# tianyili2017/HEVC-Complexity-Reduction

Measured on AMD Instinct MI355X. Metric: CTUs/sec (ETH-CNN inference), higher is better.
Workload: dtype f32; 1 GPU; All-Intra 3840x2160 QP32, 50 frames synthetic YUV; width=3840, height=2160, frames_per_gpu=50, qp=32, ranks=1, devices_visible=1, rank0_device=0, one_rank_per_device=True, device=AMD Radeon Graphics (gfx950:sramecc+:xnack-, 256 CUs), host NUMA node 0

## Files before the change

hevc-complexity-reduction_amd/csrc/ethcnn_context.cpp:

```cpp
#include "ethcnn_ctx.h"

static thread_local std::string g_create_err;

int set_err(ethcnn_ctx* c, int code, const char* fmt, ...) {
    char buf[512];
    va_list ap;
    va_start(ap, fmt);
    std::vsnprintf(buf, sizeof buf, fmt, ap);
    va_end(ap);
    if (c) c->err = buf; else g_create_err = buf;
    return code;
}

extern "C" const char* ethcnn_version(void) { return "ethcnn-mi355x 0.1 (gfx950)"; }

extern "C" const char* ethcnn_last_error(const ethcnn_ctx* ctx) {
    return ctx ? ctx->err.c_str() : g_create_err.c_str();
}

int ensure_side_streams(ethcnn_ctx* c) {
    hipStream_t* ss[] = {&c->copy_in, &c->copy_out, &c->s_tile};
    for (hipStream_t* s : ss)
        if (!*s) HIPCHK(c, hipStreamCreateWithFlags(s, hipStreamNonBlocking));
    return 0;
}

static void free_workspace(ethcnn_ctx* c) {
    Workspace& w = c->ws;
    void* ptrs[] = {w.featb, w.xs, w.xm, w.xl, w.feat, w.h1, w.h2, w.logits, w.raw, w.flags, c->xs1, c->xm1, c->xl1, c->h1_1, c->flags1};
    for (void* p : ptrs)
        if (p) (void)hipFree(p);
    w = Workspace();
    c->xs1 = c->xm1 = c->xl1 = nullptr;
    c->h1_1 = nullptr;
    c->flags1 = nullptr;
}

Workspace ws_view(const ethcnn_ctx* c, int p) {
    Workspace v = c->ws;
    if (p) {
        v.xs = c->xs1;
        v.xm = c->xm1;
        v.xl = c->xl1;
        v.h1 = c->h1_1;
        v.flags = c->flags1;
    }
    return v;
}

int ensure_workspace(ethcnn_ctx* c, int n, int chunks) {
    Workspace& w = c->ws;
    const int cap = (n + 15) / 16 * 16;
    if (cap > w.cap) {
        free_workspace(c);
        HIPCHK(c, hipMalloc((void**)&w.xs, (size_t)cap * 4096));
        HIPCHK(c, hipMalloc((void**)&w.xm, (size_t)cap * 2048));
        HIPCHK(c, hipMalloc((void**)&w.xl, (size_t)cap * 512));
        HIPCHK(c, hipMalloc((void**)&w.feat, (size_t)cap * kNFeat * 4));
        HIPCHK(c, hipMalloc((void**)&w.h1, (size_t)cap * kNVec * 4));
        HIPCHK(c, hipMalloc((void**)&w.h2, (size_t)cap * kNFc2 * 4));
        HIPCHK(c, hipMalloc((void**)&w.logits, (size_t)cap * kNOut * 4));
        HIPCHK(c, hipMalloc((void**)&w.raw, (size_t)cap * kNOut * 4));
        HIPCHK(c, hipMalloc((void**)&c->xs1, (size_t)cap * 4096));
        HIPCHK(c, hipMalloc((void**)&c->xm1, (size_t)cap * 2048));
        HIPCHK(c, hipMalloc((void**)&c->xl1, (size_t)cap * 512));
        HIPCHK(c, hipMalloc((void**)&c->h1_1, (size_t)cap * kNVec * 4));
        w.cap = cap;
    }
    if (c->fc1_plan != 0 && !w.featb)
        HIPCHK(c, hipMalloc((void**)&w.featb, (size_t)((w.cap + 31) / 32) * kFastPairBytes));
    const int words = sync_words(chunks);
    if (words > w.flags_cap) {
        if (w.flags) (void)hipFree(w.flags);
        if (c->flags1) (void)hipFree(c->flags1);
        w.flags = c->flags1 = nullptr;
        w.flags_cap = 0;
        HIPCHK(c, hipMalloc((void**)&w.flags, (size_t)words * sizeof(int)));
        HIPCHK(c, hipMalloc((void**)&c->flags1, (size_t)words * sizeof(int)));
        w.flags_cap = words;
    }
    return 0;
}

extern "C" int ethcnn_create(ethcnn_ctx** out, const ethcnn_options* opt) {
    if (!out) return set_err(nullptr, ETHCNN_ERR_ARG, "ethcnn_create: out is NULL");
    *out = nullptr;
    const auto t_enter = std::chrono::steady_clock::now();
    int ndev = 0;
    hipError_t e = hipGetDeviceCount(&ndev);
    const auto t_runtime = std::chrono::steady_clock::now();
    if (e != hipSuccess || ndev <= 0)
        return set_err(nullptr, ETHCNN_ERR_DEVICE, "no HIP device available (%s): libethcnn has no CPU fallback",
                       e == hipSuccess ? "device count 0" : hipGetErrorString(e));
    const int dev = opt ? opt->device : 0;
    if (dev < 0 || dev >= ndev) return set_err(nullptr, ETHCNN_ERR_ARG, "device %d out of range (0..%d)", dev, ndev - 1);
    std::vector<std::pair<const char*, std::chrono::steady_clock::time_point>> marks;
    auto mark = [&](const char* what) { marks.emplace_back(what, std::chrono::steady_clock::now()); };
    hipDeviceProp_t prop;
    if ((e = hipGetDeviceProperties(&prop, dev)) != hipSuccess)
        return set_err(nullptr, ETHCNN_ERR_DEVICE, "hipGetDeviceProperties: %s", hipGetErrorString(e));
    if (std::strncmp(prop.gcnArchName, "gfx950", 6) != 0)
        return set_err(nullptr, ETHCNN_ERR_DEVICE, "device %d is %s; libethcnn is built for gfx950 only", dev, prop.gcnArchName);
    ethcnn_ctx* c = new (std::nothrow) ethcnn_ctx();
    if (!c) return set_err(nullptr, ETHCNN_ERR_NOMEM, "out of memory");
    c->device = dev;
    std::snprintf(c->devname, sizeof c->devname, "%s (%s, %d CUs)", prop.name, prop.gcnArchName, prop.multiProcessorCount);
// ... 52 lines not shown
        }
        (void)hipGetLastError();
        if (qe == hipSuccess && node >= 0) {
            char path[96], buf[1024];
            std::snprintf(path, sizeof path, "/sys/devices/system/node/node%d/cpulist", node);
            if (FILE* f = std::fopen(path, "r")) {
                if (std::fgets(buf, sizeof buf, f)) {
                    CPU_ZERO(&c->numa.set);
                    int n = 0;
                    for (char* q = buf; *q && *q != '\n';) {
                        char* end;
                        const long a = std::strtol(q, &end, 10);
                        long b = a;
                        if (end == q) break;
                        if (*end == '-') { q = end + 1; b = std::strtol(q, &end, 10); }
                        for (long k = a; k <= b && k < CPU_SETSIZE; ++k) { CPU_SET((int)k, &c->numa.set); ++n; }
                        q = (*end == ',') ? end + 1 : end;
                    }
                    cpu_set_t own;
                    if (n > 0 && sched_getaffinity(0, sizeof own, &own) == 0) {
                        n = 0;
                        for (int k = 0; k < CPU_SETSIZE; ++k) {
                            if (CPU_ISSET(k, &c->numa.set) && !CPU_ISSET(k, &own)) CPU_CLR(k, &c->numa.set);
                            if (CPU_ISSET(k, &c->numa.set)) ++n;
                        }
                    }
                    c->numa.valid = n > 0;
                    if (c->numa.valid) {
                        const size_t L = std::strlen(c->devname);
                        std::snprintf(c->devname + L, sizeof c->devname - L, ", host NUMA node %d", node);
                    }
                }
                std::fclose(f);
            }
        }
    }
    if (const char* e = dev_env("ETHCNN_TILE_BLOCKS")) c->tile_blocks = std::max(1, std::atoi(e));
    mark("NUMA lookup");
    if (const char* tm = std::getenv("ETHCNN_TIMING"))
        if (std::atoi(tm) != 0) {
            std::string line = "ethcnn_create timing (ms): first HIP call (runtime init) " + std::to_string(std::chrono::duration<double, std::milli>(t_runtime - t_enter).count());
            auto prev = t_runtime;
            for (const auto& m : marks) {
                char buf[96];
                std::snprintf(buf, sizeof buf, " | %s %.2f", m.first, std::chrono::duration<double, std::milli>(m.second - prev).count());
                line += buf;
                prev = m.second;
            }
            std::fprintf(stderr, "%s\n", line.c_str());
        }
    c->startup_ms[0] = std::chrono::duration<double, std::milli>(t_runtime - t_enter).count();
    c->startup_ms[1] = std::chrono::duration<double, std::milli>(std::chrono::steady_clock::now() - t_enter).count();
    *out = c;
    return ETHCNN_OK;
}

extern "C" void ethcnn_destroy(ethcnn_ctx* c) {
    if (!c) return;
    (void)hipSetDevice(c->device);
    if ((c->ldp.open || c->ai.open) && c->h_rows)
        for (int cy = 0; cy < kStreamCtuRows; ++cy) __atomic_store_n(c->h_rows + cy, c->rows_seq, __ATOMIC_RELEASE);
    (void)hipDeviceSynchronize();
    if (c->h_done) { (void)hipHostFree(c->h_done); c->h_done = nullptr; }
    if (c->h_rows) { (void)hipHostFree(c->h_rows); c->h_rows = nullptr; }
    for (auto& p : c->pending) { c->ev_pool.push_back(p.a); c->ev_pool.push_back(p.b); }
    for (hipEvent_t e : c->ev_pool) (void)hipEventDestroy(e);
    free_workspace(c);
    free_staging(c);
    {
        std::vector<std::thread> th;
        for (ethcnn_ctx* p : c->peers)
            if (p) th.emplace_back([p] { ethcnn_destroy(p); });
        for (auto& t : th) t.join();
        c->peers.clear();
    }
    (void)hipSetDevice(c->device);
    for (const auto& r : c->pinned) (void)hipHostFree(const_cast<char*>(r.first));
    delete c->pool;
    if (c->dw_arena) (void)hipFree(c->dw_arena);
    if (c->dw_fast) (void)hipFree(c->dw_fast);
    if (c->dw_trunk16) (void)hipFree(c->dw_trunk16);
    if (c->dw_heads16) (void)hipFree(c->dw_heads16);
    {
        void* lp[] = {c->d_lstm, c->d_vec, c->d_state[0], c->d_state[1], c->d_lprobs, c->d_lgate, c->d_ssync, c->seq_vec, c->seq_probs, c->narrow_buf, c->d_compare};
        for (void* p : lp)
            if (p) (void)hipFree(p);
    }
    {
        hipEvent_t evs[] = {c->e_tile[0], c->e_tile[1], c->e_trunk[0], c->e_trunk[1], c->e_main, c->e_fc1[0], c->e_fc1[1], c->e_band[0], c->e_band[1], c->e_band[2], c->e_band[3]};
        for (hipEvent_t e : evs)
            if (e) (void)hipEventDestroy(e);
    }
    hipStream_t streams[] = {c->stream, c->copy_in, c->copy_out, c->s_tile};
    for (hipStream_t st : streams)
        if (st) (void)hipStreamDestroy(st);
    delete c;
}

extern "C" int ethcnn_get_startup_times(const ethcnn_ctx* c, double* runtime_init_ms, double* create_ms) {
    if (!c) return ETHCNN_ERR_ARG;
    if (runtime_init_ms) *runtime_init_ms = c->startup_ms[0];
    if (create_ms) *create_ms = c->startup_ms[1];
    return ETHCNN_OK;
}

extern "C" int ethcnn_device_name(const ethcnn_ctx* c, char* out, size_t cap) {
    if (!c || !out || cap == 0) return ETHCNN_ERR_ARG;
    std::snprintf(out, cap, "%s", c->devname);
    return ETHCNN_OK;
}

extern "C" int ethcnn_set_thresholds(ethcnn_ctx* c, float t1, float t2) {
    if (!c) return ETHCNN_ERR_ARG;
    c->thr1 = t1;
    c->thr2 = t2;
    return ETHCNN_OK;
}
extern "C" int ethcnn_get_thresholds(const ethcnn_ctx* c, float* t1, float* t2) {
    if (!c || !t1 || !t2) return ETHCNN_ERR_ARG;
    *t1 = c->thr1;
    *t2 = c->thr2;
    return ETHCNN_OK;
}
extern "C" int ethcnn_load_thresholds(ethcnn_ctx* c, const char* path) {
    if (!c || !path) return ETHCNN_ERR_ARG;
    char err[400];
    float a, b;
    const int rc = parse_thr_info(path, &a, &b, err, sizeof err);
    if (rc) return set_err(c, rc, "%s", err);
    c->thr1 = a;
    c->thr2 = b;
    return ETHCNN_OK;
}

hipEvent_t get_event(ethcnn_ctx* c) {
    if (!c->ev_pool.empty()) {
        hipEvent_t e = c->ev_pool.back();
        c->ev_pool.pop_back();
        return e;
    }
    hipEvent_t e = nullptr;
    if (hipEventCreate(&e) != hipSuccess) e = nullptr;
    return e;
}
static void drain_events(ethcnn_ctx* c) {
    for (auto& p : c->pending) {
        float ms = 0.f;
        if (hipEventSynchronize(p.b) == hipSuccess && hipEventElapsedTime(&ms, p.a, p.b) == hipSuccess) {
            c->times.ms[p.stage] += ms;
        } else {
            c->times.timing_errors++;
            c->times.timed[p.stage]--;
            c->times.timed_ctus[p.stage] -= p.ctus;
        }
        c->ev_pool.push_back(p.a);
        c->ev_pool.push_back(p.b);
    }
    c->pending.clear();
}
extern "C" int ethcnn_set_profiling(ethcnn_ctx* c, int on) {
    if (!c) return ETHCNN_ERR_ARG;
    drain_events(c);
    c->profiling = on < 0 ? 0 : (on > 2 ? 2 : on);
    c->fc1_sample = 0;
    return ETHCNN_OK;
}
extern "C" int ethcnn_set_pass_pipeline(ethcnn_ctx* c, int on) {
// ... 114 lines not shown
```

hevc-complexity-reduction_amd/csrc/ethcnn_ctx.h:

```cpp
#pragma once
#include <hip/hip_runtime.h>
#if defined(__SSE2__)
#include <emmintrin.h>
#endif
#include <sched.h>
#include <sys/stat.h>
#include <unistd.h>

#include <algorithm>
#include <cerrno>
#include <cstdarg>
#include <cstdio>
#include <cstdlib>
#include <cstring>
#include <atomic>
#include <chrono>
#include <condition_variable>
#include <functional>
#include <mutex>
#include <string>
#include <thread>
#include <vector>

#include "ethcnn_kernels.h"
// ... 11 lines not shown
        if (n.valid && sched_getaffinity(0, sizeof saved_, &saved_) == 0 && sched_setaffinity(0, sizeof n.set, &n.set) == 0) on_ = true;
    }
    ~AffinityScope() {
        if (on_) (void)sched_setaffinity(0, sizeof saved_, &saved_);
    }
private:
    cpu_set_t saved_;
    bool on_ = false;
};

class HostPool {
public:
    HostPool(int nthreads, const NumaCpus& numa) {
        for (int t = 1; t < nthreads; ++t)
            workers_.emplace_back([this, numa] {
                if (numa.valid) (void)sched_setaffinity(0, sizeof numa.set, &numa.set);
                loop();
            });
    }
    ~HostPool() {
        {
            std::lock_guard<std::mutex> lk(m_);
            stop_ = true;
        }
        cv_.notify_all();
        for (auto& t : workers_) t.join();
    }
    int size() const { return (int)workers_.size() + 1; }
    int run(int n, const std::function<int(int)>& fn) {
        if (n <= 0) return 0;
        if (workers_.empty() || n == 1) {
            for (int u = 0; u < n; ++u)
                if (int r = fn(u)) return r;
            return 0;
        }
        {
            std::lock_guard<std::mutex> lk(m_);
            fn_ = &fn;
            n_ = n;
            next_.store(0);
            rc_.store(0);
            pending_ = (int)workers_.size();
            ++gen_;
        }
        cv_.notify_all();
        drain();
        std::unique_lock<std::mutex> lk(m_);
        done_.wait(lk, [this] { return pending_ == 0; });
        fn_ = nullptr;
        return rc_.load();
    }

private:
    void drain() {
        for (int u = next_.fetch_add(1); u < n_ && rc_.load() == 0; u = next_.fetch_add(1))
            if (int r = (*fn_)(u)) rc_.store(r);
    }
    void loop() {
        unsigned long seen = 0;
        for (;;) {
            {
                std::unique_lock<std::mutex> lk(m_);
                cv_.wait(lk, [&] { return stop_ || gen_ != seen; });
                if (stop_) return;
                seen = gen_;
            }
            drain();
            std::lock_guard<std::mutex> lk(m_);
            if (--pending_ == 0) done_.notify_one();
        }
    }
    std::vector<std::thread> workers_;
    std::mutex m_;
    std::condition_variable cv_, done_;
    const std::function<int(int)>* fn_ = nullptr;
    std::atomic<int> next_{0}, rc_{0};
    int n_ = 0, pending_ = 0;
    unsigned long gen_ = 0;
    bool stop_ = false;
};

constexpr int kStageBufs = 4;
constexpr int kPipelineMinCtus = 8192;

struct ethcnn_ctx {
    int device = 0;
    hipStream_t stream = nullptr;
    hipStream_t copy_in = nullptr;
    hipStream_t copy_out = nullptr;
    char devname[128] = {0};
    std::string err;
    double startup_ms[2] = {0, 0};

    bool have_weights = false;
    std::vector<float> blob;
    DeviceWeights dw;
    float* dw_arena = nullptr;

    float thr1 = 0.5f, thr2 = 0.5f;

    bool have_lstm = false;
    std::vector<float> lstm_blob;
    float* d_lstm = nullptr;
    float* d_vec = nullptr;
    float* d_state[2] = {nullptr, nullptr};
    float* d_lprobs = nullptr;
    int lstm_cap = 0;
    int state_cur = -1;
    int state_nctu = 0;
    float* seq_vec = nullptr;
    float* seq_probs = nullptr;
    size_t seq_vec_cap = 0, seq_probs_cap = 0;
    int seq_chunk = 0;
    ethcnn_source_format src_fmt{8, 420};
    uint8_t* narrow_buf = nullptr;
    size_t narrow_cap = 0;
    int narrow_chunk = 0;
    std::vector<uint8_t> narrow_host;

    Workspace ws;
    uint4 *xs1 = nullptr, *xm1 = nullptr, *xl1 = nullptr;
    float* h1_1 = nullptr;
    int* flags1 = nullptr;
    hipStream_t s_tile = nullptr;
    hipEvent_t e_tile[2] = {}, e_trunk[2] = {}, e_main = nullptr;
    hipEvent_t e_fc1[2] = {};
    int tile_after_fc1 = 0;
    hipEvent_t e_band[4] = {};
    int* d_lgate = nullptr;
    int lgate_chunks = 0;
    bool lgate_clean = false;
    int lgate_n = -1;
    int lstm_epoch = 0;
    int lstm_one_launch = 1;
    int tile_blocks = 256;
    unsigned pass_idx = 0;
    int last_parity = 0;
    int small_launch = 1;
    bool luma_over_pcie = false;
    int pull = 1;
    int* d_ssync = nullptr;
    int ssync_cap = 0;
    bool ssync_clean = false;
    int small_epoch = 0;
    int fc1_plan = 0;
    uint16_t* dw_fast = nullptr;
    uint16_t* dw_trunk16 = nullptr;
    uint16_t* dw_heads16 = nullptr;
    int guard_state[4] = {0, 0, 0, 0};
    double guard_bound[4] = {0, 0, 0, 0};
    double guard_measured[4] = {-1, -1, -1, -1};
    FastGuard guard_info[4] = {};
    int last_fast = 0;
    unsigned long passes = 0, fast_passes = 0;
    bool ws_foreign = false;
    unsigned long long* d_compare = nullptr;
    unsigned* h_done = nullptr;
    unsigned* h_rows = nullptr;
    unsigned rows_seq = 1;
    const unsigned* tile_wait_rows = nullptr;
    int stream_stage_reruns = 0;
    float* host_probs = nullptr;
    bool host_probs_used = false;
    struct LdpPending { bool open = false, streamed = false; float* probs = nullptr; float* d_probs = nullptr; size_t pbytes = 0; int out = 0, in = -1, nctu = 0;
                        bool in_from_host = false; int prev_cur = -1, prev_nctu = 0; } ldp;
    struct LumaPending { bool open = false, direct = false; float* probs = nullptr; size_t out_bytes = 0; } ai;
    unsigned done_seq = 0;
    unsigned done_armed = 0;
    int done_sync = 1;
    int cus = 0;
    bool main_dirty = false;
    int overlap = 1;
    int max_ctus = kMaxCtusPerPass;
    int host_threads_opt = 0;
    int last_n = 0;
    bool debug_capture = false;

    int profiling = 0;
    unsigned fc1_sample = 0;
    struct Ev { hipEvent_t a, b; int stage; long ctus; };
    std::vector<Ev> pending;
    std::vector<hipEvent_t> ev_pool;
    ethcnn_stage_times times{};

    uint8_t* h_in[kStageBufs] = {};
    float* h_out[kStageBufs] = {};
    uint8_t* d_in[kStageBufs] = {};
    float* d_out[kStageBufs] = {};
    hipEvent_t ev_in[kStageBufs] = {}, ev_comp[kStageBufs] = {}, ev_out[kStageBufs] = {};
    size_t in_cap = 0, out_cap = 0;
    std::vector<std::pair<const char*, size_t>> pinned;
    std::vector<ethcnn_ctx*> peers;
    int shard_workers = 1;
    const ethcnn_ctx* weights_from = nullptr;
    unsigned weights_gen = 0;
    HostPool* pool = nullptr;
    NumaCpus numa;
};

constexpr int kStreamCtuRows = 1024;

int set_err(ethcnn_ctx* c, int code, const char* fmt, ...);

#define HIPCHK(c, call)                                                                       \
    do {                                                                                      \
        hipError_t e_ = (call);                                                               \
        if (e_ != hipSuccess)                                                                 \
            return set_err((c), ETHCNN_ERR_DEVICE, "%s failed: %s", #call, hipGetErrorString(e_)); \
    } while (0)

Workspace ws_view(const ethcnn_ctx* c, int p);
int ensure_workspace(ethcnn_ctx* c, int n, int chunks);
int ensure_side_streams(ethcnn_ctx* c);
hipEvent_t get_event(ethcnn_ctx* c);
int ensure_fast_weights(ethcnn_ctx* c, int plan);
int upload_lstm_image(ethcnn_ctx* c, const float* blob, float** d_image);
int calibrate_fast_plan(ethcnn_ctx* c, int plan, double* max_abs);
int make_geom(ethcnn_ctx* c, int w, int h, ptrdiff_t pitch, ptrdiff_t fstride, FrameGeom* g);
// ... 50 lines not shown
```

hevc-complexity-reduction_amd/csrc/ethcnn_kernels.h:

```cpp
#pragma once
#include <hip/hip_runtime.h>

#include "ethcnn_spec.h"

namespace ethcnn {

struct Workspace {
    int cap = 0;
    uint4* xs = nullptr;
    uint4* xm = nullptr;
    uint4* xl = nullptr;
    float* feat = nullptr;
    uint16_t* featb = nullptr;
    float* h1 = nullptr;
    float* h2 = nullptr;
    float* logits = nullptr;
    float* raw = nullptr;
    int* flags = nullptr;
    int flags_cap = 0;
};

struct FrameGeom {
    int width, height;
    long pitch, frame_stride;
    int cw, ch, nctu;
};

void launch_tile(const uint8_t* d_luma, const FrameGeom& g, long ctu0, int n, const Workspace& ws, int n_flags,
                 hipStream_t s, int max_blocks = 0, const unsigned* wait_rows = nullptr, unsigned wait_seq = 0, unsigned* gave_up = nullptr);
void launch_trunk(const Workspace& ws, const DeviceWeights& w, int n, bool resi, hipStream_t s, int fc1_plan = 0);
void launch_trunk_f16(const Workspace& ws, const DeviceWeights& w, int n, hipStream_t s);
void launch_trunk_f16_foldall(const uint8_t* d_luma, const FrameGeom& g, long ctu0, int n, const Workspace& ws, const DeviceWeights& w, int n_flags,
                              hipStream_t s);
void launch_fc1(const Workspace& ws, const DeviceWeights& w, int n, float* out, hipStream_t s);
void launch_fc1_fast(const Workspace& ws, const DeviceWeights& w, int n, float* out, int plan, hipStream_t s, int cus = 256);
void launch_heads(const Workspace& ws, const DeviceWeights& w, int n, float qn, int nctu_per_frame,
                  long ctu0, float thr1, float thr2, float* d_probs, hipStream_t s);
void launch_heads_f16(const Workspace& ws, const DeviceWeights& w, int n, float qn, int nctu_per_frame, long ctu0, float thr1, float thr2,
                      float* d_probs, hipStream_t s);
#ifdef ETHCNN_FULL_FENCE
#define ETHCNN_HANDOFF_RELEASE() asm volatile("buffer_wbl2 sc1\n\ts_waitcnt vmcnt(0) lgkmcnt(0)" ::: "memory")
#define ETHCNN_HANDOFF_ACQUIRE() asm volatile("buffer_inv sc1" ::: "memory")
#else
#define ETHCNN_HANDOFF_RELEASE() asm volatile("s_waitcnt vmcnt(0)" ::: "memory")
#define ETHCNN_HANDOFF_ACQUIRE() \
    do {                         \
    } while (0)
#endif

inline int sync_words(int nchunks) { return 2 * nchunks + 8; }
constexpr int kSmallPassMaxCtus = 2304;
bool small_pass_ok(const uint8_t* d_luma, const FrameGeom& g, int n);
int small_pass_sync_words(int n, int nchunks);
void launch_small_pass(const uint8_t* d_luma, const FrameGeom& g, long ctu0, int n, bool resi, const Workspace& ws,
                       const DeviceWeights& w, float* fc1_out, float qn, float thr1, float thr2, float* d_probs, int nchunks,
                       int* d_sync, int epoch, unsigned* done, unsigned done_seq, hipStream_t s, bool pull = false,
                       const unsigned* wait_rows = nullptr, unsigned wait_seq = 0, unsigned* gave_up = nullptr, float* host_probs = nullptr);
void launch_gate(const Workspace& ws, int n, int nctu_per_frame, long ctu0, float thr2, float* d_probs,
                 hipStream_t s);

unsigned lstm_heads_blocks(int n);
int lstm_gate_words(int n);
void launch_lstm(const float* d_vec, const float* d_state_in, float* d_state_out, const float* d_lstm_blob, int n, int qp,
                 int i_frame, float thr1, float thr2, float* d_raw, float* d_probs, int* d_gate, unsigned* done, unsigned done_seq,
                 int one_launch, int epoch, hipStream_t s);
int lstm_frame_words(int n);
constexpr int kLstmOneLaunchMaxCtus = 640;

void launch_mfma_rate(int blocks, int iters, float* d_sink, hipStream_t s);

int chunks_per_frame(int nctu);

struct GateIndex {
    int nctu, cpf, r0, c0;
    float inv_nctu;
};
__device__ __forceinline__ int gate_chunk(const GateIndex& gi, int ctu) {
    const int u = gi.r0 + ctu;
    int f = (int)((float)u * gi.inv_nctu);
    if (f * gi.nctu > u) --f;
    if ((f + 1) * gi.nctu <= u) ++f;
    return f * gi.cpf + (u - f * gi.nctu) / kSubBatch - gi.c0;
}

inline GateIndex make_gate_index(int nctu, long ctu0) {
    GateIndex gi;
    gi.nctu = nctu;
    gi.cpf = chunks_per_frame(nctu);
    gi.r0 = (int)(ctu0 % nctu);
    gi.c0 = gi.r0 / kSubBatch;
    gi.inv_nctu = 1.0f / (float)nctu;
    return gi;
}


}
```

hevc-complexity-reduction_amd/csrc/ethcnn_kernels.hip:

```cpp
#include <hip/hip_runtime.h>

#include <cstdlib>

#include "ethcnn_kernels.h"

namespace ethcnn {

int chunks_per_frame(int nctu) { return (nctu + kSubBatch - 1) / kSubBatch; }


__global__ __launch_bounds__(256) void k5_gate(float* __restrict__ probs, const int* __restrict__ flags, int N,
                                               GateIndex gi, float thr2) {
    const int idx = blockIdx.x * 256 + threadIdx.x;
    const int i = idx / kNOut, j = idx % kNOut;
    if (i >= N || j == 0) return;
    const int chunk = gate_chunk(gi, i);
    const bool open32 = flags[2 * chunk] != 0;
    const bool open16 = open32 ? (flags[2 * chunk + 1] != 0) : (0.0f > thr2);
    if (j < 5 ? !open32 : !open16) probs[(size_t)i * kNOut + j] = 0.0f;
}

void launch_gate(const Workspace& ws, int n, int nctu, long ctu0, float thr2, float* d_probs, hipStream_t s) {
    const long total = (long)n * kNOut;
    hipLaunchKernelGGL(k5_gate, dim3((unsigned)((total + 255) / 256)), dim3(256), 0, s, d_probs, ws.flags, n,
                       make_gate_index(nctu, ctu0), thr2);
}

typedef float f32x4_cal __attribute__((ext_vector_type(4)));
__global__ __launch_bounds__(256) void k_mfma_rate(int iters, float* sink) {
    f32x4_cal acc[4] = {{0.f, 0.f, 0.f, 0.f}, {0.f, 0.f, 0.f, 0.f}, {0.f, 0.f, 0.f, 0.f}, {0.f, 0.f, 0.f, 0.f}};
    const float a = 1.0f + threadIdx.x * 1e-7f, b = 0.999f;
    for (int i = 0; i < iters; ++i) {
#pragma unroll
        for (int u = 0; u < 8; ++u)
#pragma unroll
            for (int j = 0; j < 4; ++j) acc[j] = __builtin_amdgcn_mfma_f32_16x16x4f32(a, b, acc[j], 0, 0, 0);
    }
    const float s = acc[0][0] + acc[1][1] + acc[2][2] + acc[3][3];
    if (s == 123.456f) *sink = s;
}
void launch_mfma_rate(int blocks, int iters, float* d_sink, hipStream_t s) {
    hipLaunchKernelGGL(k_mfma_rate, dim3(blocks), dim3(256), 0, s, iters, d_sink);
}

}
```

hevc-complexity-reduction_amd/csrc/ethcnn_pass.cpp:

```cpp
#include "ethcnn_ctx.h"

int make_geom(ethcnn_ctx* c, int w, int h, ptrdiff_t pitch, ptrdiff_t fstride, FrameGeom* g) {
    if (w <= 0 || h <= 0) return set_err(c, ETHCNN_ERR_ARG, "bad frame size %dx%d", w, h);
    if (pitch < w) return set_err(c, ETHCNN_ERR_ARG, "pitch %td < width %d", pitch, w);
    g->width = w;
    g->height = h;
    g->pitch = (long)pitch;
    g->frame_stride = (long)fstride;
    g->cw = (w + 63) / 64;
    g->ch = (h + 63) / 64;
    g->nctu = g->cw * g->ch;
    return 0;
}

unsigned done_arm(ethcnn_ctx* c) {
    if (!c->done_sync || !c->h_done) return 0;
    if (++c->done_seq == 0) ++c->done_seq;
    return c->done_seq;
}
hipError_t stream_sync(ethcnn_ctx* c) {
    const unsigned seq = c->done_armed;
    c->done_armed = 0;
    if (seq) {
        const auto t0 = std::chrono::steady_clock::now();
        for (unsigned spins = 1;; ++spins) {
            if (__atomic_load_n(c->h_done, __ATOMIC_ACQUIRE) == seq) return hipSuccess;
#if defined(__SSE2__)
            _mm_pause();
#endif
            if ((spins & 4095u) == 0 && std::chrono::steady_clock::now() - t0 > std::chrono::milliseconds(5)) break;
        }
    }
    return hipStreamSynchronize(c->stream);
}

int serial_end(ethcnn_ctx* c) {
    c->main_dirty = true;
    return 0;
}

int run_small_pass(ethcnn_ctx* c, const uint8_t* d_luma, const FrameGeom& g, long ctu0, int n, bool resi, const Workspace& w,
                   float* fc1_out, float qn, float* d_probs, int nchunks, bool pull, const unsigned* wait_rows) {
    const int words = small_pass_sync_words(n, nchunks);
    c->done_armed = 0;
    if (c->small_epoch >= (1 << 30)) c->ssync_clean = false;
    if (words > c->ssync_cap || !c->ssync_clean) {
        if (words > c->ssync_cap) {
            HIPCHK(c, hipStreamSynchronize(c->stream));
            if (c->d_ssync) (void)hipFree(c->d_ssync);
            c->d_ssync = nullptr;
            c->ssync_cap = 0;
            const int cap = words;
            HIPCHK(c, hipMalloc((void**)&c->d_ssync, (size_t)cap * sizeof(int)));
            c->ssync_cap = cap;
        }
        HIPCHK(c, hipMemsetAsync(c->d_ssync, 0, (size_t)c->ssync_cap * sizeof(int), c->stream));
        c->small_epoch = 0;
    }
    ++c->small_epoch;
    c->ssync_clean = false;
    (void)hipGetLastError();
    const unsigned seq = resi ? 0u : done_arm(c);
    { StageTimer t(c, ETHCNN_STAGE_FC1, n); launch_small_pass(d_luma, g, ctu0, n, resi, w, c->dw, fc1_out, qn, c->thr1, c->thr2, d_probs, nchunks, c->d_ssync, c->small_epoch, seq ? c->h_done : nullptr, seq, c->stream, pull, wait_rows, c->rows_seq, c->h_done + 1, (seq && !resi) ? c->host_probs : nullptr); }
    const hipError_t le = hipGetLastError();
    if (le != hipSuccess) return set_err(c, ETHCNN_ERR_DEVICE, "launch of the single-launch small pass failed: %s", hipGetErrorString(le));
    c->ssync_clean = true;
    c->done_armed = seq;
    c->host_probs_used = seq && !resi && c->host_probs != nullptr && reinterpret_cast<uintptr_t>(c->host_probs) % 16 == 0;
    return 0;
}

int run_pass(ethcnn_ctx* c, const uint8_t* d_luma, const FrameGeom& g, long ctu0, int n, int qp, float* d_probs_pass,
             hipEvent_t input_ready) {
    const int cpf = chunks_per_frame(g.nctu);
    const long nchunks = (ctu0 + n - 1) / g.nctu * cpf + ((ctu0 + n - 1) % g.nctu) / kSubBatch + 1 -
                         (ctu0 / g.nctu * cpf + (ctu0 % g.nctu) / kSubBatch);
    c->done_armed = 0;
    const bool takes_small = c->small_launch && n < kPipelineMinCtus && small_pass_ok(d_luma, g, n);
    int rc = (c->fc1_plan && !takes_small) ? ensure_fast_weights(c, c->fc1_plan) : 0;
    if (rc) return rc;
    rc = ensure_workspace(c, n, (int)nchunks);
    if (rc) return rc;
    const float qn = (float)qp * (1.0f / 51.0f);
    const int fast = c->fc1_plan;
    const bool foldall = fast == 3 && c->tile_wait_rows == nullptr;
    const bool side_tile = c->overlap != 0 && n >= kPipelineMinCtus && !foldall;
    const int p = side_tile ? (int)(c->pass_idx++ & 1) : 0;
    const Workspace w = ws_view(c, p);
    if (side_tile && !c->s_tile && (rc = ensure_side_streams(c)) != 0) return rc;
    hipStream_t s_tile = side_tile ? c->s_tile : c->stream;
    if (input_ready) HIPCHK(c, hipStreamWaitEvent(s_tile, input_ready, 0));
    Workspace wv = w;
    if (!c->debug_capture) wv.h2 = wv.logits = wv.raw = nullptr;
    const bool small = !side_tile && c->small_launch && small_pass_ok(d_luma, g, n);
    if (small) {
        rc = run_small_pass(c, d_luma, g, ctu0, n, false, wv, w.h1, qn, d_probs_pass, (int)nchunks, c->luma_over_pcie,
                            c->luma_over_pcie ? c->tile_wait_rows : nullptr);
        if (rc) return rc;
    } else {
        if (side_tile) {
            HIPCHK(c, hipStreamWaitEvent(s_tile, c->e_trunk[p], 0));
            if (c->main_dirty) {
                HIPCHK(c, hipEventRecord(c->e_main, c->stream));
                c->main_dirty = false;
            }
            HIPCHK(c, hipStreamWaitEvent(s_tile, c->e_main, 0));
            const bool behind_fc1 = c->tile_after_fc1 != 0 && fast != 0;
            HIPCHK(c, hipStreamWaitEvent(s_tile, behind_fc1 ? c->e_fc1[p ^ 1] : c->e_trunk[p ^ 1], 0));
        }
        (void)hipGetLastError();
#define LAUNCH_OK(name)                                                                                            \
    do {                                                                                                           \
        const hipError_t le_ = hipGetLastError();                                                                  \
        if (le_ != hipSuccess) return set_err(c, ETHCNN_ERR_DEVICE, "launch of the %s stage failed: %s", name, hipGetErrorString(le_)); \
    } while (0)
        if (!foldall) {
            StageTimer t(c, ETHCNN_STAGE_TILE, n, s_tile);
            launch_tile(d_luma, g, ctu0, n, w, sync_words((int)nchunks), s_tile, side_tile ? c->tile_blocks : 0,
                        side_tile ? nullptr : c->tile_wait_rows, c->rows_seq, c->h_done + 1);
        }
        LAUNCH_OK("tile");
        if (side_tile) {
            HIPCHK(c, hipEventRecord(c->e_tile[p], s_tile));
            HIPCHK(c, hipStreamWaitEvent(c->stream, c->e_tile[p], 0));
        }
        {
            StageTimer t(c, ETHCNN_STAGE_TRUNK);
            if (foldall) launch_trunk_f16_foldall(d_luma, g, ctu0, n, w, c->dw, sync_words((int)nchunks), c->stream);
            else if (fast == 3) launch_trunk_f16(w, c->dw, n, c->stream);
            else launch_trunk(w, c->dw, n, false, c->stream, fast);
        }
        LAUNCH_OK("trunk");
        if (side_tile) HIPCHK(c, hipEventRecord(c->e_trunk[p], c->stream));
        if (fast) {
            { StageTimer t(c, ETHCNN_STAGE_FC1, n); launch_fc1_fast(w, c->dw, n, w.h1, 2, c->stream, c->cus); }
            LAUNCH_OK("FC1 (16-bit pipe)");
            if (side_tile && c->tile_after_fc1) HIPCHK(c, hipEventRecord(c->e_fc1[p], c->stream));
        } else {
            { StageTimer t(c, ETHCNN_STAGE_FC1, n); launch_fc1(w, c->dw, n, w.h1, c->stream); }
            LAUNCH_OK("FC1");
        }
        {
            StageTimer t(c, ETHCNN_STAGE_HEADS);
            if (fast == 3 && c->dw.heads16_w) launch_heads_f16(wv, c->dw, n, qn, g.nctu, ctu0, c->thr1, c->thr2, d_probs_pass, c->stream);
            else launch_heads(wv, c->dw, n, qn, g.nctu, ctu0, c->thr1, c->thr2, d_probs_pass, c->stream);
        }
        { StageTimer t(c, ETHCNN_STAGE_GATE); launch_gate(w, n, g.nctu, ctu0, c->thr2, d_probs_pass, c->stream); }
        LAUNCH_OK("heads / gate");
#undef LAUNCH_OK
    }
    if (!side_tile) c->main_dirty = true;
    c->times.ctus += n;
    c->last_n = n;
    c->last_parity = p;
    c->last_fast = small ? 0 : fast;
    ++c->passes;
    c->ws_foreign = false;
    if (c->last_fast) ++c->fast_passes;
    return 0;
}

std::vector<Pass> plan_passes(int nctu, int nframes, int max_ctus) {
    std::vector<Pass> out;
    if (nctu <= max_ctus) {
        const int fpp = std::max(1, max_ctus / nctu);
        for (int f = 0; f < nframes; f += fpp) {
            const int nf = std::min(fpp, nframes - f);
            out.push_back({(long)f * nctu, nf * nctu});
        }
    } else {
        for (int f = 0; f < nframes; ++f)
            for (int o = 0; o < nctu; o += max_ctus) out.push_back({(long)f * nctu + o, std::min(max_ctus, nctu - o)});
    }
    return out;
}

static void calibration_picture(std::vector<uint8_t>& luma, int w, int h) {
    luma.resize((size_t)w * h);
    uint64_t s = 0x9E3779B97F4A7C15ull;
    auto rnd = [&]() { s ^= s << 13; s ^= s >> 7; s ^= s << 17; return (uint32_t)(s >> 32); };
    for (int ty = 0; ty < h / 128; ++ty)
        for (int tx = 0; tx < w / 128; ++tx) {
            const int kind = (tx + 5 * ty) % 6, base = 16 + (int)(rnd() % 208), amp = 1 + (int)(rnd() % 6), per = 4 << (rnd() % 4);
            for (int y = 0; y < 128; ++y)
                for (int x = 0; x < 128; ++x) {
                    int v;
                    switch (kind) {
                        case 0: v = base; break;
                        case 1: v = base + (int)(rnd() % (2 * amp + 1)) - amp; break;
                        case 2: v = (x * 2 + y) % 256; break;
                        case 3: v = (int)(rnd() & 255); break;
                        case 4: v = ((x / per) & 1) ? 235 : 20; break;
                        default: { const int a = x % (2 * per), b = y % (2 * per);
                                   v = 128 + (a < per ? a : 2 * per - a) * 96 / per - 48 + (b < per ? b : 2 * per - b) * 32 / per - 16; }
                    }
                    luma[(size_t)(ty * 128 + y) * w + tx * 128 + x] = (uint8_t)std::min(255, std::max(0, v));
                }
        }
}
int calibrate_fast_plan(ethcnn_ctx* c, int plan, double* max_abs) {
    constexpr int W = 2048, H = 1280;
    constexpr int kQps[2] = {22, 37};
    FrameGeom g;
    int rc = make_geom(c, W, H, W, (ptrdiff_t)W * H, &g);
    if (rc) return rc;
    std::vector<uint8_t> luma;
    calibration_picture(luma, W, H);
    const size_t pf = (size_t)g.nctu * kNOut;
    uint8_t* d_luma = nullptr;
    float* d_p = nullptr;
    HIPCHK(c, hipMalloc((void**)&d_luma, luma.size()));
    if (hipMalloc((void**)&d_p, 4 * pf * 4) != hipSuccess) { (void)hipFree(d_luma); return set_err(c, ETHCNN_ERR_NOMEM, "calibration: out of device memory"); }
    std::vector<float> p(4 * pf);
    const float t1 = c->thr1, t2 = c->thr2;
    const int plan0 = c->fc1_plan, small0 = c->small_launch;
    const bool cap0 = c->debug_capture, pcie0 = c->luma_over_pcie;
    const unsigned* const wait0 = c->tile_wait_rows;
    float* const hp0 = c->host_probs;
    c->thr1 = c->thr2 = -1.0f;
    c->small_launch = 0;
    c->debug_capture = false;
    c->tile_wait_rows = nullptr;
    c->luma_over_pcie = false;
    c->host_probs = nullptr;
    hipError_t e = hipMemcpyAsync(d_luma, luma.data(), luma.size(), hipMemcpyHostToDevice, c->stream);
    for (int k = 0; k < 4 && rc == 0 && e == hipSuccess; ++k) {
        c->fc1_plan = (k & 1) == 0 ? 0 : plan;
        rc = run_pass(c, d_luma, g, 0, g.nctu, kQps[k >> 1], d_p + k * pf);
    }
    c->thr1 = t1; c->thr2 = t2; c->fc1_plan = plan0; c->small_launch = small0; c->debug_capture = cap0;
    c->tile_wait_rows = wait0; c->luma_over_pcie = pcie0; c->host_probs = hp0;
// ... 32 lines not shown
```

hevc-complexity-reduction_amd/csrc/ethcnn_tile.hip:

```cpp
#include <hip/hip_runtime.h>

#include "ethcnn_kernels.h"
#include "ethcnn_tile_group.h"

namespace ethcnn {

template <bool FAST, bool WAIT>
__global__ __launch_bounds__(256) void k0_tile_slab(const uint8_t* __restrict__ luma, int width, int height, long pitch,
                                                    long frame_stride, int cw, int nctu, long ctu0, int n_total,
                                                    uint4* __restrict__ XS, uint4* __restrict__ XM,
                                                    uint4* __restrict__ XL, int* __restrict__ gate_flags, int n_flags, TileWait tw) {
    __shared__ uint32_t tile[16 * kSlabCtuPitch];
    if (blockIdx.x == 0)
        for (int i = threadIdx.x; i < n_flags; i += 256) gate_flags[i] = 0;
    const int ngroups = (n_total + 15) >> 4;
#pragma unroll 1
    for (int grp = blockIdx.x; grp < ngroups; grp += gridDim.x) {
        if (WAIT) tile_wait_rows(tw, ctu0, grp, n_total, nctu, cw);
        tile_group<FAST, false, false>(tile, luma, width, height, pitch, frame_stride, cw, nctu, ctu0, n_total, grp, XS, XM, XL);
    }
}

void launch_tile(const uint8_t* d_luma, const FrameGeom& g, long ctu0, int n, const Workspace& ws, int n_flags,
                 hipStream_t s, int max_blocks, const unsigned* wait_rows, unsigned wait_seq, unsigned* gave_up) {
    const int blocks = (n + 15) / 16;
    const bool fast = (g.width % 16 == 0) && (g.pitch % 16 == 0) && (g.frame_stride % 16 == 0) &&
                      (reinterpret_cast<uintptr_t>(d_luma) % 16 == 0);
    const int sb = max_blocks > 0 ? (blocks < max_blocks ? blocks : max_blocks) : blocks;
    const TileWait tw{wait_rows, wait_seq, gave_up};
    if (wait_rows && fast)
        hipLaunchKernelGGL((k0_tile_slab<true, true>), dim3(sb), dim3(256), 0, s, d_luma, g.width, g.height, g.pitch,
                           g.frame_stride, g.cw, g.nctu, ctu0, n, ws.xs, ws.xm, ws.xl, ws.flags, n_flags, tw);
    else if (wait_rows)
        hipLaunchKernelGGL((k0_tile_slab<false, true>), dim3(sb), dim3(256), 0, s, d_luma, g.width, g.height, g.pitch,
                           g.frame_stride, g.cw, g.nctu, ctu0, n, ws.xs, ws.xm, ws.xl, ws.flags, n_flags, tw);
    else if (fast)
        hipLaunchKernelGGL((k0_tile_slab<true, false>), dim3(sb), dim3(256), 0, s, d_luma, g.width, g.height, g.pitch,
                           g.frame_stride, g.cw, g.nctu, ctu0, n, ws.xs, ws.xm, ws.xl, ws.flags, n_flags, tw);
    else
        hipLaunchKernelGGL((k0_tile_slab<false, false>), dim3(sb), dim3(256), 0, s, d_luma, g.width, g.height, g.pitch,
                           g.frame_stride, g.cw, g.nctu, ctu0, n, ws.xs, ws.xm, ws.xl, ws.flags, n_flags, tw);
}

}
```

Measured before the change: 41.88 million CTU/s.

## Share tile work between side stream and main stream via atomic ticket

The tiling stage on the side stream now hands out CTU groups through a device-side atomic ticket counter. A finisher kernel launched on the main stream picks up the remaining groups, so idle CUs can help finish tiling instead of waiting on the limited-size side-stream grid. The gate kernel resets the ticket for the next pass. This adds atomic traffic, an extra launch, and reset and dirty-state logic with host synchronisation on error paths.

```diff
diff --git a/hevc-complexity-reduction_amd/csrc/ethcnn_context.cpp b/hevc-complexity-reduction_amd/csrc/ethcnn_context.cpp
--- a/hevc-complexity-reduction_amd/csrc/ethcnn_context.cpp
+++ b/hevc-complexity-reduction_amd/csrc/ethcnn_context.cpp
@@ -22,6 +22,16 @@
     hipStream_t* ss[] = {&c->copy_in, &c->copy_out, &c->s_tile};
     for (hipStream_t* s : ss)
         if (!*s) HIPCHK(c, hipStreamCreateWithFlags(s, hipStreamNonBlocking));
+    if (!c->d_tile_ticket) {
+        int* t = nullptr;
+        HIPCHK(c, hipMalloc((void**)&t, 2 * kTicketStride * sizeof(int)));
+        const hipError_t e = hipMemset(t, 0, 2 * kTicketStride * sizeof(int));
+        if (e != hipSuccess) {
+            (void)hipFree(t);
+            return set_err(c, ETHCNN_ERR_DEVICE, "cannot zero the tile ticket words: %s", hipGetErrorString(e));
+        }
+        c->d_tile_ticket = t;
+    }
     return 0;
 }
 
@@ -240,7 +250,7 @@
     if (c->dw_trunk16) (void)hipFree(c->dw_trunk16);
     if (c->dw_heads16) (void)hipFree(c->dw_heads16);
     {
-        void* lp[] = {c->d_lstm, c->d_vec, c->d_state[0], c->d_state[1], c->d_lprobs, c->d_lgate, c->d_ssync, c->seq_vec, c->seq_probs, c->narrow_buf, c->d_compare};
+        void* lp[] = {c->d_lstm, c->d_vec, c->d_state[0], c->d_state[1], c->d_lprobs, c->d_lgate, c->d_ssync, c->seq_vec, c->seq_probs, c->narrow_buf, c->d_compare, c->d_tile_ticket};
         for (void* p : lp)
             if (p) (void)hipFree(p);
     }
diff --git a/hevc-complexity-reduction_amd/csrc/ethcnn_ctx.h b/hevc-complexity-reduction_amd/csrc/ethcnn_ctx.h
--- a/hevc-complexity-reduction_amd/csrc/ethcnn_ctx.h
+++ b/hevc-complexity-reduction_amd/csrc/ethcnn_ctx.h
@@ -117,6 +117,7 @@
 
 constexpr int kStageBufs = 4;
 constexpr int kPipelineMinCtus = 8192;
+constexpr int kTicketStride = 16;
 
 struct ethcnn_ctx {
     int device = 0;
@@ -169,6 +170,8 @@
     int lstm_epoch = 0;
     int lstm_one_launch = 1;
     int tile_blocks = 256;
+    int* d_tile_ticket = nullptr;
+    bool ticket_dirty = false;
     unsigned pass_idx = 0;
     int last_parity = 0;
     int small_launch = 1;
diff --git a/hevc-complexity-reduction_amd/csrc/ethcnn_kernels.h b/hevc-complexity-reduction_amd/csrc/ethcnn_kernels.h
--- a/hevc-complexity-reduction_amd/csrc/ethcnn_kernels.h
+++ b/hevc-complexity-reduction_amd/csrc/ethcnn_kernels.h
@@ -28,6 +28,10 @@
 
 void launch_tile(const uint8_t* d_luma, const FrameGeom& g, long ctu0, int n, const Workspace& ws, int n_flags,
                  hipStream_t s, int max_blocks = 0, const unsigned* wait_rows = nullptr, unsigned wait_seq = 0, unsigned* gave_up = nullptr);
+void launch_tile_side(const uint8_t* d_luma, const FrameGeom& g, long ctu0, int n, const Workspace& ws, int n_flags, hipStream_t s,
+                      int max_blocks, int* ticket);
+bool launch_tile_finish(const uint8_t* d_luma, const FrameGeom& g, long ctu0, int n, const Workspace& ws, hipStream_t s,
+                        int max_blocks, int cus, int* ticket);
 void launch_trunk(const Workspace& ws, const DeviceWeights& w, int n, bool resi, hipStream_t s, int fc1_plan = 0);
 void launch_trunk_f16(const Workspace& ws, const DeviceWeights& w, int n, hipStream_t s);
 void launch_trunk_f16_foldall(const uint8_t* d_luma, const FrameGeom& g, long ctu0, int n, const Workspace& ws, const DeviceWeights& w, int n_flags,
@@ -57,7 +61,7 @@
                        int* d_sync, int epoch, unsigned* done, unsigned done_seq, hipStream_t s, bool pull = false,
                        const unsigned* wait_rows = nullptr, unsigned wait_seq = 0, unsigned* gave_up = nullptr, float* host_probs = nullptr);
 void launch_gate(const Workspace& ws, int n, int nctu_per_frame, long ctu0, float thr2, float* d_probs,
-                 hipStream_t s);
+                 hipStream_t s, int* reset_ticket = nullptr);
 
 unsigned lstm_heads_blocks(int n);
 int lstm_gate_words(int n);
diff --git a/hevc-complexity-reduction_amd/csrc/ethcnn_kernels.hip b/hevc-complexity-reduction_amd/csrc/ethcnn_kernels.hip
--- a/hevc-complexity-reduction_amd/csrc/ethcnn_kernels.hip
+++ b/hevc-complexity-reduction_amd/csrc/ethcnn_kernels.hip
@@ -9,8 +9,10 @@
 int chunks_per_frame(int nctu) { return (nctu + kSubBatch - 1) / kSubBatch; }
 
 
+template <bool TICKET>
 __global__ __launch_bounds__(256) void k5_gate(float* __restrict__ probs, const int* __restrict__ flags, int N,
-                                               GateIndex gi, float thr2) {
+                                               GateIndex gi, float thr2, int* __restrict__ ticket) {
+    if (TICKET && blockIdx.x == 0 && threadIdx.x == 0) *ticket = 0;
     const int idx = blockIdx.x * 256 + threadIdx.x;
     const int i = idx / kNOut, j = idx % kNOut;
     if (i >= N || j == 0) return;
@@ -20,10 +22,13 @@
     if (j < 5 ? !open32 : !open16) probs[(size_t)i * kNOut + j] = 0.0f;
 }
 
-void launch_gate(const Workspace& ws, int n, int nctu, long ctu0, float thr2, float* d_probs, hipStream_t s) {
+void launch_gate(const Workspace& ws, int n, int nctu, long ctu0, float thr2, float* d_probs, hipStream_t s, int* reset_ticket) {
     const long total = (long)n * kNOut;
-    hipLaunchKernelGGL(k5_gate, dim3((unsigned)((total + 255) / 256)), dim3(256), 0, s, d_probs, ws.flags, n,
-                       make_gate_index(nctu, ctu0), thr2);
+    const dim3 grid((unsigned)((total + 255) / 256));
+    if (reset_ticket)
+        hipLaunchKernelGGL(k5_gate<true>, grid, dim3(256), 0, s, d_probs, ws.flags, n, make_gate_index(nctu, ctu0), thr2, reset_ticket);
+    else
+        hipLaunchKernelGGL(k5_gate<false>, grid, dim3(256), 0, s, d_probs, ws.flags, n, make_gate_index(nctu, ctu0), thr2, (int*)nullptr);
 }
 
 typedef float f32x4_cal __attribute__((ext_vector_type(4)));
diff --git a/hevc-complexity-reduction_amd/csrc/ethcnn_pass.cpp b/hevc-complexity-reduction_amd/csrc/ethcnn_pass.cpp
--- a/hevc-complexity-reduction_amd/csrc/ethcnn_pass.cpp
+++ b/hevc-complexity-reduction_amd/csrc/ethcnn_pass.cpp
@@ -87,9 +87,16 @@
     const bool side_tile = c->overlap != 0 && n >= kPipelineMinCtus && !foldall;
     const int p = side_tile ? (int)(c->pass_idx++ & 1) : 0;
     const Workspace w = ws_view(c, p);
-    if (side_tile && !c->s_tile && (rc = ensure_side_streams(c)) != 0) return rc;
+    if (side_tile && (!c->s_tile || !c->d_tile_ticket) && (rc = ensure_side_streams(c)) != 0) return rc;
     hipStream_t s_tile = side_tile ? c->s_tile : c->stream;
     if (input_ready) HIPCHK(c, hipStreamWaitEvent(s_tile, input_ready, 0));
+    int* const ticket = side_tile ? c->d_tile_ticket + kTicketStride * p : nullptr;
+    if (side_tile && c->ticket_dirty) {
+        (void)hipStreamSynchronize(c->s_tile);
+        (void)hipStreamSynchronize(c->stream);
+        HIPCHK(c, hipMemset(c->d_tile_ticket, 0, 2 * kTicketStride * sizeof(int)));
+        c->ticket_dirty = false;
+    }
     Workspace wv = w;
     if (!c->debug_capture) wv.h2 = wv.logits = wv.raw = nullptr;
     const bool small = !side_tile && c->small_launch && small_pass_ok(d_luma, g, n);
@@ -114,15 +121,30 @@
         const hipError_t le_ = hipGetLastError();                                                                  \
         if (le_ != hipSuccess) return set_err(c, ETHCNN_ERR_DEVICE, "launch of the %s stage failed: %s", name, hipGetErrorString(le_)); \
     } while (0)
-        if (!foldall) {
-            StageTimer t(c, ETHCNN_STAGE_TILE, n, s_tile);
-            launch_tile(d_luma, g, ctu0, n, w, sync_words((int)nchunks), s_tile, side_tile ? c->tile_blocks : 0,
-                        side_tile ? nullptr : c->tile_wait_rows, c->rows_seq, c->h_done + 1);
-        }
-        LAUNCH_OK("tile");
         if (side_tile) {
+            c->ticket_dirty = true;
+            {
+                StageTimer t(c, ETHCNN_STAGE_TILE, n, s_tile);
+                launch_tile_side(d_luma, g, ctu0, n, w, sync_words((int)nchunks), s_tile, c->tile_blocks, ticket);
+            }
+            LAUNCH_OK("tile");
             HIPCHK(c, hipEventRecord(c->e_tile[p], s_tile));
+            if (input_ready) HIPCHK(c, hipStreamWaitEvent(c->stream, input_ready, 0));
+            if (c->profiling >= 2) {
+                StageTimer t(c, ETHCNN_STAGE_TILE, 0);
+                launch_tile_finish(d_luma, g, ctu0, n, w, c->stream, c->tile_blocks, c->cus, ticket);
+            } else {
+                launch_tile_finish(d_luma, g, ctu0, n, w, c->stream, c->tile_blocks, c->cus, ticket);
+            }
+            LAUNCH_OK("tile finisher");
             HIPCHK(c, hipStreamWaitEvent(c->stream, c->e_tile[p], 0));
+        } else {
+            if (!foldall) {
+                StageTimer t(c, ETHCNN_STAGE_TILE, n, s_tile);
+                launch_tile(d_luma, g, ctu0, n, w, sync_words((int)nchunks), s_tile, 0, c->tile_wait_rows, c->rows_seq,
+                            c->h_done + 1);
+            }
+            LAUNCH_OK("tile");
         }
         {
             StageTimer t(c, ETHCNN_STAGE_TRUNK);
@@ -145,8 +167,9 @@
             if (fast == 3 && c->dw.heads16_w) launch_heads_f16(wv, c->dw, n, qn, g.nctu, ctu0, c->thr1, c->thr2, d_probs_pass, c->stream);
             else launch_heads(wv, c->dw, n, qn, g.nctu, ctu0, c->thr1, c->thr2, d_probs_pass, c->stream);
         }
-        { StageTimer t(c, ETHCNN_STAGE_GATE); launch_gate(w, n, g.nctu, ctu0, c->thr2, d_probs_pass, c->stream); }
+        { StageTimer t(c, ETHCNN_STAGE_GATE); launch_gate(w, n, g.nctu, ctu0, c->thr2, d_probs_pass, c->stream, ticket); }
         LAUNCH_OK("heads / gate");
+        if (side_tile) c->ticket_dirty = false;
 #undef LAUNCH_OK
     }
     if (!side_tile) c->main_dirty = true;
diff --git a/hevc-complexity-reduction_amd/csrc/ethcnn_tile.hip b/hevc-complexity-reduction_amd/csrc/ethcnn_tile.hip
--- a/hevc-complexity-reduction_amd/csrc/ethcnn_tile.hip
+++ b/hevc-complexity-reduction_amd/csrc/ethcnn_tile.hip
@@ -19,6 +19,82 @@
         if (WAIT) tile_wait_rows(tw, ctu0, grp, n_total, nctu, cw);
         tile_group<FAST, false, false>(tile, luma, width, height, pitch, frame_stride, cw, nctu, ctu0, n_total, grp, XS, XM, XL);
     }
+}
+
+template <bool FAST, bool SIDE>
+__global__ __launch_bounds__(256) void k0_tile_ticket(const uint8_t* __restrict__ luma, int width, int height, long pitch,
+                                                      long frame_stride, int cw, int nctu, long ctu0, int n_total,
+                                                      uint4* __restrict__ XS, uint4* __restrict__ XM, uint4* __restrict__ XL,
+                                                      int* __restrict__ gate_flags, int n_flags, int* __restrict__ ticket, int side_groups) {
+    __shared__ uint32_t tile[16 * kSlabCtuPitch];
+    __shared__ int s_ticket;
+    if (SIDE && blockIdx.x == 0)
+        for (int i = threadIdx.x; i < n_flags; i += 256) gate_flags[i] = 0;
+    const int ngroups = (n_total + 15) >> 4;
+    int grp = SIDE ? (int)blockIdx.x : ngroups;
+    if (!SIDE) {
+        if (threadIdx.x == 0) s_ticket = __hip_atomic_load(ticket, __ATOMIC_RELAXED, __HIP_MEMORY_SCOPE_AGENT);
+        __syncthreads();
+        const int v = s_ticket;
+        __syncthreads();
+        if (v < 0 || v >= ngroups - side_groups - (int)blockIdx.x) return;
+    }
+#pragma unroll 1
+    for (;;) {
+        if (grp < ngroups)
+            tile_group<FAST, false, false>(tile, luma, width, height, pitch, frame_stride, cw, nctu, ctu0, n_total, grp, XS, XM, XL);
+        if (threadIdx.x == 0) s_ticket = __hip_atomic_fetch_add(ticket, 1, __ATOMIC_RELAXED, __HIP_MEMORY_SCOPE_AGENT);
+        __syncthreads();
+        const int t = s_ticket;
+        __syncthreads();
+        if (t < 0 || t >= ngroups - side_groups) break;
+        grp = side_groups + t;
+    }
+}
+
+template <bool SIDE>
+static void launch_ticket(const uint8_t* d_luma, const FrameGeom& g, long ctu0, int n, const Workspace& ws, int n_flags, hipStream_t s,
+                          int blocks, int* ticket, int side_groups) {
+    const bool fast = (g.width % 16 == 0) && (g.pitch % 16 == 0) && (g.frame_stride % 16 == 0) &&
+                      (reinterpret_cast<uintptr_t>(d_luma) % 16 == 0);
+    if (fast)
+        hipLaunchKernelGGL((k0_tile_ticket<true, SIDE>), dim3(blocks), dim3(256), 0, s, d_luma, g.width, g.height, g.pitch,
+                           g.frame_stride, g.cw, g.nctu, ctu0, n, ws.xs, ws.xm, ws.xl, ws.flags, n_flags, ticket, side_groups);
+    else
+        hipLaunchKernelGGL((k0_tile_ticket<false, SIDE>), dim3(blocks), dim3(256), 0, s, d_luma, g.width, g.height, g.pitch,
+                           g.frame_stride, g.cw, g.nctu, ctu0, n, ws.xs, ws.xm, ws.xl, ws.flags, n_flags, ticket, side_groups);
+}
+
+int tile_side_groups(int n, int max_blocks) {
+    const int groups = (n + 15) / 16;
+    return groups < max_blocks ? groups : max_blocks;
+}
+
+void launch_tile_side(const uint8_t* d_luma, const FrameGeom& g, long ctu0, int n, const Workspace& ws, int n_flags, hipStream_t s,
+                      int max_blocks, int* ticket) {
+    const int sb = tile_side_groups(n, max_blocks);
+    launch_ticket<true>(d_luma, g, ctu0, n, ws, n_flags, s, sb, ticket, sb);
+}
+
+static int tile_blocks_per_cu() {
+    static const int per_cu = [] {
+        int b = 0;
+        if (hipOccupancyMaxActiveBlocksPerMultiprocessor(&b, k0_tile_ticket<true, false>, 256, 0) != hipSuccess || b < 1) {
+            (void)hipGetLastError();
+            b = 4;
+        }
+        return b < 8 ? b : 8;
+    }();
+    return per_cu;
+}
+
+bool launch_tile_finish(const uint8_t* d_luma, const FrameGeom& g, long ctu0, int n, const Workspace& ws, hipStream_t s,
+                        int max_blocks, int cus, int* ticket) {
+    const int side = tile_side_groups(n, max_blocks), left = (n + 15) / 16 - side;
+    if (left <= 0) return false;
+    const int full = cus * tile_blocks_per_cu();
+    launch_ticket<false>(d_luma, g, ctu0, n, ws, 0, s, left < full ? left : full, ticket, side);
+    return true;
 }
 
 void launch_tile(const uint8_t* d_luma, const FrameGeom& g, long ctu0, int n, const Workspace& ws, int n_flags,
```

Result: no change. 42.04 million CTU/s, median of 6 (+0.4%).
